# jianing-sun/Mask-YOLO

Hardware: AMD Instinct MI355X
Metric: images/sec fwd+bwd, 224x224 Shapes batch 32, at 1 MI355X (higher is better)
Workload: dtype f32

## Files before the change

### include/myolo_hip_internal.h

```cpp
#ifndef MYOLO_HIP_INTERNAL_H
#define MYOLO_HIP_INTERNAL_H

#include "myolo_hip.h"

#ifdef __cplusplus
extern "C" {
#endif

int myolo_bn_frozen_coeffs_batched(const float* params, const float* stats, const int64_t* table, int nlayers, float* coeffs,
                                   void* stream);

int myolo_bn_act_bwd_frozen_post(const float* dy, const float* a_post, const float* gamma, const float* beta, const float* scale,
                                 float* dx, float* dgamma, float* dbeta, int64_t M, int C, int act,
                                 void* ws, size_t ws_bytes, void* stream);

int myolo_wprep_create(void* arena, size_t arena_bytes, void** handle);
int myolo_wprep_destroy(void* h);
int myolo_wprep_activate(void* h);
int myolo_wprep_count(void* h);
int myolo_wprep_invalidate(void* h);
int myolo_wprep_refresh(void* h, int first, int last, int max_idle, void* stream);
int myolo_wprep_stats(void* h, long long* hits, long long* misses, long long* bytes_used);
int myolo_wprep_overflows(void* h, long long* n);

// ... 81 lines not shown

int myolo_gemm_tn_bf16x6_planes(const float* A, const float* B, float* C, int nruns, const int64_t* rows, const int32_t* nq, int Ka, int N,
                                void* ws, size_t ws_bytes, void* stream);
int myolo_deconv2x2s2_bwd_weight_bf16x6(const float* x, const float* dy, float* dw, int N, int H, int W, int Cin, int Cout, void* ws, size_t ws_bytes,
                                        void* stream);

size_t myolo_wino63_bwd_data_ws_bytes(int N, int Cin, int Cout);
int myolo_wino63_bwd_data_lazybn(const float* y_pre, const float* dy_compact, const int32_t* inv, const float* scale, const float* shift,
                                 const float* ka, const float* kb, int act, const float* w, float* dx, int N, int Cin, int Cout, void* ws,
                                 size_t ws_bytes, void* stream);
int myolo_conv3x3s2_c3_affine_act_fwd(const float* x, const float* w, const float* scale, const float* shift, int act, float* y,
                                      int N, int H, int W, int Cout, void* stream);
size_t myolo_conv3x3s2_c3_bnstats_ws_bytes(int N, int H, int W, int Cout);
int myolo_conv3x3s2_c3_bnstats_fwd(const float* x, const float* w, float* y, const float* gamma, const float* beta, float* mean, float* var,
                                   float* scale, float* shift, float* moving_mean, float* moving_var, int N, int H, int W, int Cout, int phases,
                                   void* ws, size_t ws_bytes, void* stream);
size_t myolo_dwconv3x3_bnstats_ws_bytes(int N, int H, int W, int C, int stride);
int myolo_dwconv3x3_bnstats_fwd(const float* x, const float* in_scale, const float* in_shift, int in_act, const float* w, float* y,
                                const float* gamma, const float* beta, float* mean, float* var, float* scale, float* shift,
                                float* moving_mean, float* moving_var, int N, int H, int W, int C, int stride, int phases,
                                void* ws, size_t ws_bytes, void* stream);
int myolo_dwconv3x3_bwd_weight_affine_in(const float* x, const float* in_scale, const float* in_shift, int in_act, const float* dy, float* dw,
                                         int N, int H, int W, int C, int stride, void* ws, size_t ws_bytes, void* stream);
int    myolo_pwconv1x1_bnstats_ok(int Cin, int Cout);
size_t myolo_pwconv1x1_bnstats_ws_bytes(int64_t M, int Cin, int Cout);
int myolo_pwconv1x1_bnstats_fwd(const float* x, const float* in_scale, const float* in_shift, int in_act, const float* w, float* y,
                                const float* gamma, const float* beta, float* mean, float* var, float* scale, float* shift,
                                float* moving_mean, float* moving_var, int64_t M, int Cin, int Cout, int phases, void* ws, size_t ws_bytes, void* stream);
int myolo_pwconv1x1_bwd_weight_affine_in(const float* x, const float* in_scale, const float* in_shift, int in_act, const float* dy, float* dw,
                                         int64_t M, int Cin, int Cout, void* ws, size_t ws_bytes, void* stream);

int myolo_mask_bce_sel(const float* target_masks, const int32_t* target_class_ids, const float* pred, float loss_weight,
                       float* loss_out, float* dz_sel, int NR, int h, int w, int C, void* ws, size_t ws_bytes, void* stream);
size_t myolo_mask_head_out_bwd_sel_ws_bytes(int NR, int Cin);
int myolo_mask_head_out_bwd_sel(const float* x, const float* w, const float* dz_sel, const int32_t* ids, float* dx, float* dw, float* db,
                                int64_t M, int Cin, int C, int hw, void* ws, size_t ws_bytes, void* stream);

int myolo_stream_copy(const void* src, void* dst, size_t nbytes, int variant, int blocks, void* stream);
int myolo_mfma_probe(int kind, int iters, int blocks, float* out, void* stream);

size_t myolo_conv7x7s2_c3_ws_bytes(int N, int H, int W, int Cout);
int myolo_conv7x7s2_c3_fwd(const float* x, const float* w, const float* bias, float* y, int N, int H, int W, int Cout,
                           void* ws, size_t ws_bytes, void* stream);
int myolo_conv7x7s2_c3_bnstats_fwd(const float* x, const float* w, const float* bias, float* y, const float* gamma, const float* beta, float* mean,
                                   float* var, float* scale, float* shift, float* moving_mean, float* moving_var, int N, int H, int W, int Cout,
                                   void* ws, size_t ws_bytes, void* stream);
// ... 116 lines not shown
```

### mask-yolo_amd/csrc/mem_kernels.hip

```cpp
#include "myolo_common.h"
#include <type_traits>
#include <stdlib.h>
#include <stdarg.h>
#include <string.h>

static thread_local char g_err[512] = "";
extern "C" void myolo_set_error(const char* fmt, ...)
{
    va_list ap;
    va_start(ap, fmt);
    vsnprintf(g_err, sizeof(g_err), fmt, ap);
    va_end(ap);
}
extern "C" const char* myolo_last_error_string(void) { return g_err; }
extern "C" int myolo_version(void) { return 213; }

static MyoloOptions default_options() { MyoloOptions o = {}; o.bn_fused_tf_variance = 1; o.tn_wgs = 224; return o; }
MyoloOptions g_myolo_opt = default_options();
static int* option_slot(const char* name)
{
    static const struct { const char* n; int MyoloOptions::*m; } tab[] = {
        {"gemm_generic", &MyoloOptions::gemm_generic}, {"no_splitk", &MyoloOptions::no_splitk}, {"bf16_no256", &MyoloOptions::bf16_no256},
        {"bf16_force256", &MyoloOptions::bf16_force256}, {"bf16_no_c3", &MyoloOptions::bf16_no_c3}, {"bf16_no_loopn", &MyoloOptions::bf16_no_loopn},
        {"bf16_mask_valu", &MyoloOptions::bf16_mask_valu}, {"bf16_mask_nofin", &MyoloOptions::bf16_mask_nofin},
// ... 316 lines not shown

struct OpStats {
    static constexpr int NV = 2;
    const float* x;
    int C;
    __device__ void operator()(long long r, int c, float4* acc) const
    {
        const float4 v = ld4g(x + r * C + c);
        acc[0].x += v.x; acc[0].y += v.y; acc[0].z += v.z; acc[0].w += v.w;
        acc[1] = f4fma(v, v, acc[1]);
    }
};

struct FinBnStats {
    static constexpr int PAIR = 1;
    const float* gamma;
    const float* beta;
    float *mean, *var, *scale, *shift, *mmean, *mvar;
    double M;
    int fused_tf;
    __device__ void operator()(int, double) const {}
    __device__ void pair(int c, double sum, double sumsq) const
    {
        const double mu = sum / M;
        double vr = sumsq / M - mu * mu;
        if (vr < 0) vr = 0;
        const float rstd = (float)(1.0 / sqrt(vr + (double)BN_EPS_F));
        const float sc = gamma[c] * rstd;
        mean[c] = (float)mu;
        var[c] = (float)vr;
        scale[c] = sc;
        shift[c] = beta[c] - (float)mu * sc;
        if (mmean) {
            float vb = (float)vr;
            if (fused_tf && M > 1.0) vb = vb * ((float)M / ((float)M - 1.0f));
            const float vu = vb * ((float)M / ((float)M - (1.0f + BN_EPS_F)));
            mmean[c] = mmean[c] * BN_MOMENTUM_F + (float)mu * (1.0f - BN_MOMENTUM_F);
            mvar[c] = mvar[c] * BN_MOMENTUM_F + vu * (1.0f - BN_MOMENTUM_F);
        }
    }
};

__global__ void bn_frozen_kernel(const float* gamma, const float* beta, const float* mm, const float* mv,
                                 float* scale, float* shift, int C)
{
    const int c = blockIdx.x * blockDim.x + threadIdx.x;
    if (c >= C) return;
    const float rstd = (float)(1.0 / sqrt((double)mv[c] + (double)BN_EPS_F));
    const float sc = gamma[c] * rstd;
    scale[c] = sc;
    shift[c] = beta[c] - mm[c] * sc;
}

__global__ __launch_bounds__(256) void bn_frozen_batched_kernel(const float* __restrict__ params, const float* __restrict__ stats,
                                                                const long long* __restrict__ table, float* __restrict__ coeffs)
// ... 1111 lines not shown
            double d0 = 0, d1 = 0, d2 = 0, d3 = 0;
            for (int j = 0; j < PX; ++j) {
                const float4 tt = red[j * CQB + tid];
                d0 += tt.x; d1 += tt.y; d2 += tt.z; d3 += tt.w;
            }
            double* o = part + (blk * 9 + v) * C + (cb * CQB + tid) * 4;
            o[0] = d0; o[1] = d1; o[2] = d2; o[3] = d3;
        }
    }
}

template <int S, int CQB>
static void dw_rows_launch(const DwRowsGeom& g, const float* x, const float* w, float* y, int H, int W, int C, DwAffine af, DwFuse fu, hipStream_t s,
                           bool flip = false)
{
    const unsigned xcd = (g.tiles % 8 == 0 && g.tiles >= 64) ? (unsigned)(g.tiles / 8) : 0u;
    const int flags = flip ? 8 : 0;
#define DW_ROWS_GO(MODE, R6) hipLaunchKernelGGL((dw_rows_kernel<S, CQB, MODE, R6>), dim3((unsigned)g.tiles), dim3(256), 0, s, x, w, y, H, W, C, H / S, W / S, g.strips, g.chunks, g.rc, g.ncb, xcd, flags, af, fu)
    if (fu.bw.x) { if constexpr (S == 1) DW_ROWS_GO(3, false); }
    else if (fu.in.scale || fu.stat) { if (fu.in.scale && fu.in.act == MYOLO_ACT_RELU6) DW_ROWS_GO(1, true); else DW_ROWS_GO(1, false); }
    else if (af.scale) { if (af.act == MYOLO_ACT_RELU6) DW_ROWS_GO(2, true); else DW_ROWS_GO(2, false); }
    else DW_ROWS_GO(0, false);
#undef DW_ROWS_GO
}

template <int S>
__global__ __launch_bounds__(256) void dw_bwd_data_kernel(const float* __restrict__ dy, const float* __restrict__ w,
                                                          float* __restrict__ dx, int N, int H, int W, int C, int Ho, int Wo)
{
    const int pt = (S == 1) ? 1 : 0;
    const int cq = C / 4;
    const unsigned e = blockIdx.x * blockDim.x + threadIdx.x;
    if (e >= (unsigned)(W * cq)) return;
    const int ix = e / (unsigned)cq;
    const int c = (e - ix * cq) * 4;
    const int iy = blockIdx.y, n = blockIdx.z;
    float4 acc = f4zero();
#pragma unroll
    for (int ky = 0; ky < 3; ++ky) {
        const int ty = iy + pt - ky;
        if (ty < 0 || (ty % S) != 0) continue;
        const int oy = ty / S;
        if (oy >= Ho) continue;
#pragma unroll
        for (int kx = 0; kx < 3; ++kx) {
            const int tx = ix + pt - kx;
// ... 1547 lines not shown
        double* part = (double*)ws;
        double* tot = (double*)((char*)ws + align256((size_t)nblk * 2 * C * sizeof(double)));
        if (phases & 1) {
            const int rc = dw_fwd_launch(x, w, y, N, H, W, C, stride, DwAffine{nullptr, nullptr, MYOLO_ACT_NONE}, stream, DwFuse{in, part});
            if (rc != MYOLO_OK) return rc;
        }
        if (phases & 2) hipLaunchKernelGGL((colreduce_finish<FinBnStats>), dim3((C + 3) / 4), dim3(256), 0, s, part, tot, nblk, 2 * C, C, fin);
    } else {
        if (phases & 1) {
            const int rc = dw_fwd_launch(x, w, y, N, H, W, C, stride, DwAffine{nullptr, nullptr, MYOLO_ACT_NONE}, stream, DwFuse{in, nullptr});
            if (rc != MYOLO_OK) return rc;
        }
        if (phases & 2) {
            double* part = (double*)ws;
            double* tot = (double*)((char*)ws + align256(col_ws_bytes(M, C, 2)));
            OpStats op{y, C};
            run_colreduce(op, M, C, part, tot, s, fin);
        }
    }
    MYOLO_CHECK_LAUNCH();
    return MYOLO_OK;
}

int myolo_dwconv3x3_bwd_data_bnsums_rows(int N, int H, int W, int C, int stride)
{
    if (N <= 0 || (C & 3)) return 0;
    if (stride == 1) return dw_rows_ok(H, W, C) ? dw_rows_geom(N, H, W, C, 1).nblk : 0;
    if (stride != 2 || (H & 1) || (W & 1)) return 0;
    const int cq = C / 4;
    const long long total = (long long)N * (H / 2) * (W / 2) * cq;
    if (cq > 256 || (256 % cq) != 0 || total >= (1ll << 31) * 256) return 0;
    if (cq > 64) return 0;
    return (int)((total + 255) / 256);
}

static int dw_bwd_data_impl(const float* dy, const float* w, float* dx, int N, int H, int W, int C, int stride, DwBnBwd bw, void* stream);

int myolo_dwconv3x3_bwd_data(const float* dy, const float* w, float* dx, int N, int H, int W, int C, int stride, void* stream)
{
    return dw_bwd_data_impl(dy, w, dx, N, H, W, C, stride, DwBnBwd{nullptr, nullptr, nullptr, nullptr, nullptr, 0, nullptr}, stream);
}

int myolo_dwconv3x3_bwd_data_bnsums(const float* dy, const float* w, float* dx, int N, int H, int W, int C, int stride, const float* xbn,
                                    const float* scale, const float* shift, const float* mean, const float* var, int act, double* part, int rows,
                                    void* stream)
{
// ... 357 lines not shown
```

### mask-yolo_amd/myolo/_ext.py

```python
import ctypes
import os

import torch

_LIB = None
_HERE = os.path.dirname(os.path.abspath(__file__))
LIB_PATH = os.environ.get("MYOLO_LIB") or os.path.join(_HERE, "_lib", "libmyolo_hip.so")

P, I, L, F, Z, D = ctypes.c_void_p, ctypes.c_int, ctypes.c_int64, ctypes.c_float, ctypes.c_size_t, ctypes.c_double

SIGS = {
    "myolo_conv3x3s2_c3_fwd": [P, P, P, I, I, I, I, P],
    "myolo_conv3x3s2_c3_affine_act_fwd": [P, P, P, P, I, P, I, I, I, I, P],
    "myolo_conv3x3s2_c3_bwd_weight": [P, P, P, I, I, I, I, P, Z, P],
    "myolo_dwconv3x3_fwd": [P, P, P, I, I, I, I, I, P],
    "myolo_dwconv3x3_affine_act_fwd": [P, P, P, P, I, P, I, I, I, I, I, P],
    "myolo_dwconv3x3_bwd_data": [P, P, P, I, I, I, I, I, P],
    "myolo_dwconv3x3_bwd_data_bnsums": [P, P, P, I, I, I, I, I, P, P, P, P, P, I, P, I, P],
    "myolo_bn_act_bwd_from_partials": [P, P, P, P, P, P, P, P, P, L, I, I, P, I, P, Z, P],
    "myolo_dwconv3x3_bwd_weight": [P, P, P, I, I, I, I, I, P, Z, P],
    "myolo_pwconv1x1_fwd": [P, P, P, P, L, I, I, P, Z, P],
    "myolo_pwconv1x1_affine_act_fwd": [P, P, P, P, I, P, L, I, I, P, Z, P],
    "myolo_bn_frozen_coeffs_batched": [P, P, P, I, P, P],
    "myolo_pwconv1x1_bwd_data": [P, P, P, L, I, I, P, Z, P],
# ... 62 lines not shown
    "myolo_conv3x3_wino_bwd_data_lazybn": [P, P, P, P, P, P, P, I, P, P, I, I, I, I, I, P, Z, P],
    "myolo_conv3x3_wino_bwd_weight_lazybn": [P, P, P, P, P, P, P, P, I, P, I, I, I, I, I, P, Z, P],
    "myolo_wino_input_transform_roialign": [P, P, P, P, I, I, I, I, I, I, I, P],
    "myolo_pack_weights_bf16": [P, I, I, I, P, P, P, P, P, P, P, P],
    "myolo_crop_and_resize_bf16_fwd": [P, P, P, P, I, I, I, I, I, I, I, P],
    "myolo_conv3x3_bf16_fwd": [P, P, P, P, I, I, I, I, I, I, P],
    "myolo_deconv2x2s2_bf16_fwd": [P, P, P, P, I, I, I, I, I, I, P],
    "myolo_deconv2x2s2_mask_bf16_fwd": [P, P, P, P, P, P, I, I, I, I, I, I, P, Z, P],
    "myolo_mask_head_out_bf16_fwd": [P, P, P, P, L, I, I, P],
    "myolo_mask_head_out_bwd": [P, P, P, P, P, P, L, I, I, P, Z, P],
    "myolo_mask_bce": [P, P, P, F, P, P, I, I, I, I, P, Z, P],
    "myolo_mask_bce_sel": [P, P, P, F, P, P, I, I, I, I, P, Z, P],
    "myolo_mask_head_out_bwd_sel": [P, P, P, P, P, P, P, L, I, I, I, P, Z, P],
    "myolo_adam_step": [P, P, P, P, L, F, F, F, F, F, P],
    "myolo_grad_sumsq": [P, P, L, F, F, P, P, P],
    "myolo_adamw_ema_step": [P, P, P, P, P, P, L, P, F, F, F, F, F, F, F, F, P],
    "myolo_swap_f32": [P, P, L, P],
    "myolo_matmul_f32": [P, P, P, L, I, I, I, I, P, Z, P],
    "myolo_stream_copy": [P, P, Z, I, I, P],
    "myolo_mfma_probe": [I, I, I, P, P],
    "myolo_conv3x3s2_c3_bnstats_fwd": [P, P, P, P, P, P, P, P, P, P, P, I, I, I, I, I, P, Z, P],
    "myolo_dwconv3x3_bnstats_fwd": [P, P, P, I, P, P, P, P, P, P, P, P, P, P, I, I, I, I, I, I, P, Z, P],
    "myolo_dwconv3x3_bwd_weight_affine_in": [P, P, P, I, P, P, I, I, I, I, I, P, Z, P],
    "myolo_pwconv1x1_bnstats_fwd": [P, P, P, I, P, P, P, P, P, P, P, P, P, P, L, I, I, I, P, Z, P],
    "myolo_pwconv1x1_bwd_weight_affine_in": [P, P, P, I, P, P, L, I, I, P, Z, P],
    "myolo_gemm_tn_bf16x6_planes": [P, P, P, I, P, P, I, I, P, Z, P],
    "myolo_deconv2x2s2_bwd_weight_bf16x6": [P, P, P, I, I, I, I, I, P, Z, P],
    "myolo_gather_groups_affine_act": [P, P, P, P, I, P, P, I, L, I, P],
    "myolo_add_inplace": [P, P, L, P],
    "myolo_conv7x7s2_c3_fwd": [P, P, P, P, I, I, I, I, P, Z, P],
    "myolo_conv7x7s2_c3_bnstats_fwd": [P, P, P, P, P, P, P, P, P, P, P, P, I, I, I, I, P, Z, P],
    "myolo_conv7x7s2_c3_affine_act_fwd": [P, P, P, P, P, I, P, I, I, I, I, P, Z, P],
    "myolo_conv7x7s2_c3_bwd_weight": [P, P, P, P, I, I, I, I, P, Z, P],
    "myolo_maxpool3x3s2_fwd": [P, P, P, I, P, P, I, I, I, I, P],
    "myolo_maxpool3x3s2_bwd": [P, P, P, I, I, I, I, P],
    "myolo_gather_s2": [P, P, I, I, I, I, P],
    "myolo_scatter_s2": [P, P, P, I, I, I, I, P],
    "myolo_residual_fwd": [P, P, P, P, P, P, P, L, I, P],
    "myolo_residual_bwd": [P, P, P, L, P],
    "myolo_fill": [P, F, L, P],
    "myolo_u8_to_unit_f32": [P, P, L, P],
    "myolo_augment_batch": [P, P, P, P, D, P, P, P, P, P, P, P, I, I, I, I, I, I, I, P, Z, P],
    "myolo_mosaic_batch": [P, P, P, P, P, P, D, P, P, P, P, P, P, P, P, I, I, I, I, I, I, I, P, Z, P],
    "myolo_copy_paste_batch": [P, P, P, P, P, P, P, P, P, P, P, P, P, I, I, I, I, I, I, I, P, Z, P],
    "myolo_segment_masks": [P, P, P, P, P, P, P, P, P, P, I, I, I, I, P],
    "myolo_resize_images_u8": [P, Z, P, P, P, P, I, I, I, P, Z, P],
# ... 16 lines not shown
    global _LIB
    if _LIB is not None:
        return _LIB
    if not os.path.exists(LIB_PATH):
        raise RuntimeError("libmyolo_hip.so not built (%s): run `python __graft_entry__.py` "
                           "(hipcc --offload-arch=gfx950); there is no fallback path" % LIB_PATH)
    lib = ctypes.CDLL(LIB_PATH)
    for name, argtypes in SIGS.items():
        fn = getattr(lib, name)
        fn.argtypes = argtypes
        fn.restype = ctypes.c_int
    lib.myolo_version.restype = ctypes.c_int
    lib.myolo_last_error_string.restype = ctypes.c_char_p
    lib.myolo_workspace_bytes.argtypes = [L, I, I]
    lib.myolo_workspace_bytes.restype = Z
    lib.myolo_conv3x3_wino_ws_bytes.argtypes = [I, I, I, I, I, I]
    lib.myolo_conv3x3_wino_ws_bytes.restype = Z
    lib.myolo_matmul_f32_ws_bytes.argtypes = [I, I, I, I]
    lib.myolo_matmul_f32_ws_bytes.restype = Z
    lib.myolo_conv3x3s2_c3_bnstats_ws_bytes.argtypes = [I, I, I, I]
    lib.myolo_conv3x3s2_c3_bnstats_ws_bytes.restype = Z
    lib.myolo_dwconv3x3_bnstats_ws_bytes.argtypes = [I, I, I, I, I]
    lib.myolo_dwconv3x3_bnstats_ws_bytes.restype = Z
    lib.myolo_dwconv3x3_bwd_weight_ws_bytes.argtypes = [I, I, I, I, I]
    lib.myolo_dwconv3x3_bwd_weight_ws_bytes.restype = Z
    lib.myolo_pwconv1x1_bnstats_ws_bytes.argtypes = [L, I, I]
    lib.myolo_pwconv1x1_bnstats_ws_bytes.restype = Z
    lib.myolo_pwconv1x1_bnstats_ok.argtypes = [I, I]
    lib.myolo_pwconv1x1_bnstats_ok.restype = I
    lib.myolo_wino_plane_elems.argtypes = [I, I, I, I]
    lib.myolo_wino_plane_elems.restype = Z
    lib.myolo_wino_u_elems.argtypes = [I, I]
    lib.myolo_wino_u_elems.restype = Z
    lib.myolo_wino63_u_elems.argtypes = [I, I]
    lib.myolo_wino63_u_elems.restype = Z
    lib.myolo_wino63_plane_elems.argtypes = [I, I]
    lib.myolo_wino63_plane_elems.restype = Z
    lib.myolo_wino63_bwd_data_ws_bytes.argtypes = [I, I, I]
    lib.myolo_wino63_bwd_data_ws_bytes.restype = Z
    lib.myolo_conv3x3_wino63_ws_bytes.argtypes = [I, I, I, I]
    lib.myolo_conv3x3_wino63_ws_bytes.restype = Z
    lib.myolo_wino63_bwd_weight_ws_bytes.argtypes = [I, I, I]
    lib.myolo_wino63_bwd_weight_ws_bytes.restype = Z
    for fn in (lib.myolo_wino63_bwd_data_from_v_ws_bytes, lib.myolo_wino63_bwd_weight_from_q_ws_bytes):
        fn.argtypes = [I, I, I]
        fn.restype = Z
# ... 20 lines not shown
    lib.myolo_conv7x7s2_c3_ws_bytes.restype = Z
    lib.myolo_augment_batch_ws_bytes.argtypes = [I, I]
    lib.myolo_augment_batch_ws_bytes.restype = Z
    lib.myolo_mosaic_batch_ws_bytes.argtypes = [I, I]
    lib.myolo_mosaic_batch_ws_bytes.restype = Z
    lib.myolo_copy_paste_batch_ws_bytes.argtypes = [I, I]
    lib.myolo_copy_paste_batch_ws_bytes.restype = Z
    lib.myolo_resize_images_ws_bytes.argtypes = [I]
    lib.myolo_resize_images_ws_bytes.restype = Z
    lib.myolo_rle_masks_ws_bytes.argtypes = [I, I, I]
    lib.myolo_rle_masks_ws_bytes.restype = Z
    lib.myolo_contour_masks_ws_bytes.argtypes = [I, I, I, I, L]
    lib.myolo_contour_masks_ws_bytes.restype = Z
    lib.myolo_anchor_kmeans_ws_bytes.argtypes = [L, I]
    lib.myolo_anchor_kmeans_ws_bytes.restype = Z
    lib.myolo_wprep_refresh.argtypes = [P, I, I, I, P]
    lib.myolo_wprep_refresh.restype = I
    _LIB = lib
    return lib


def exported_symbols():
    return list(SIGS) + ["myolo_version", "myolo_last_error_string", "myolo_workspace_bytes", "myolo_conv3x3_wino_ws_bytes", "myolo_wino_plane_elems", "myolo_wino_u_elems", "myolo_wino63_u_elems", "myolo_wino63_plane_elems", "myolo_wino63_ok", "myolo_wino63_bwd_data_ws_bytes", "myolo_wino63_bwd_weight_ws_bytes", "myolo_wino63_bwd_data_from_v_ws_bytes", "myolo_wino63_bwd_weight_from_q_ws_bytes", "myolo_wino63_output_transform_bn_ws_bytes", "myolo_conv3x3_wino63_ws_bytes", "myolo_matmul_f32_ws_bytes", "myolo_conv3x3s2_c3_bnstats_ws_bytes", "myolo_dwconv3x3_bnstats_ws_bytes", "myolo_dwconv3x3_bwd_weight_ws_bytes",
                              "myolo_pwconv1x1_bnstats_ws_bytes", "myolo_pwconv1x1_bnstats_ok",
                              "myolo_deconv2x2s2_mask_ws_bytes", "myolo_wino_output_transform_bn_ws_bytes", "myolo_mask_head_out_bwd_sel_ws_bytes",
                              "myolo_dwconv3x3_bwd_data_bnsums_rows", "myolo_wprep_create", "myolo_wprep_destroy", "myolo_wprep_activate", "myolo_wprep_invalidate", "myolo_wprep_count", "myolo_wprep_refresh",
                              "myolo_conv7x7s2_c3_ws_bytes", "myolo_augment_batch_ws_bytes", "myolo_mosaic_batch_ws_bytes", "myolo_copy_paste_batch_ws_bytes",
                              "myolo_resize_images_ws_bytes",
                              "myolo_rle_masks_ws_bytes", "myolo_contour_masks_ws_bytes", "myolo_anchor_kmeans_ws_bytes"]


def ptr(t):
    if t is None:
        return None
    assert t.is_cuda and t.is_contiguous(), "C-ABI needs contiguous device tensors"
    return t.data_ptr()


def stream():
    return torch.cuda.current_stream().cuda_stream


def call(name, *args):
    lib = load()
    rc = getattr(lib, name)(*args)
    if rc != 0:
        raise RuntimeError("%s failed (%d): %s" % (name, rc, lib.myolo_last_error_string().decode()))
# ... 191 lines not shown
def anchor_kmeans_ws_bytes(n, runs):
    return int(load().myolo_anchor_kmeans_ws_bytes(int(n), int(runs)))


def workspace_bytes(rows, cin, cout):
    return int(load().myolo_workspace_bytes(int(rows), int(cin), int(cout)))


def wino_ws_bytes(n, h, w, cin, cout, which):
    return int(load().myolo_conv3x3_wino_ws_bytes(int(n), int(h), int(w), int(cin), int(cout), int(which)))


PRODUCTS_NATIVE, PRODUCTS_BF16X6 = 0, 1


def conv1_bnstats_ws_bytes(n, h, w, cout):
    return int(load().myolo_conv3x3s2_c3_bnstats_ws_bytes(int(n), int(h), int(w), int(cout)))


def dw_bnstats_ws_bytes(n, h, w, c, stride):
    return int(load().myolo_dwconv3x3_bnstats_ws_bytes(int(n), int(h), int(w), int(c), int(stride)))


def dw_bwd_weight_ws_bytes(n, h, w, c, stride):
    return int(load().myolo_dwconv3x3_bwd_weight_ws_bytes(int(n), int(h), int(w), int(c), int(stride)))


def pw_bnstats_ws_bytes(m, cin, cout):
    return int(load().myolo_pwconv1x1_bnstats_ws_bytes(int(m), int(cin), int(cout)))


def pw_bnstats_ok(cin, cout):
    return bool(load().myolo_pwconv1x1_bnstats_ok(int(cin), int(cout)))


def matmul_ws_bytes(k, n, b_is_nk, products):
    return int(load().myolo_matmul_f32_ws_bytes(int(k), int(n), int(b_is_nk), int(products)))


def wino_u_elems(cin, cout):
    return int(load().myolo_wino_u_elems(int(cin), int(cout)))


def dw_bwd_data_bnsums_rows(n, h, w, c, stride):
    return int(load().myolo_dwconv3x3_bwd_data_bnsums_rows(int(n), int(h), int(w), int(c), int(stride)))

# ... 52 lines not shown
```

### mask-yolo_amd/myolo/engine.py

```python
import contextlib
import gc
import os
import threading
import time

import numpy as np
import torch

from . import _ext as X

ACT_NONE, ACT_RELU, ACT_RELU6 = 0, 1, 2

BACKBONE_BLOCKS = [(64, 1), (64, 2), (128, 1), (256, 2), (256, 1), (512, 1)]
YOLO_BLOCKS = [(512, 2), (512, 1), (512, 1), (512, 1), (512, 1), (512, 1), (1024, 2), (1024, 1)]
MASK_FILTERS = 256
RESNET_STAGES = [(2, "abc", (64, 64, 256), 1), (3, "abcd", (128, 128, 512), 2), (4, "abcdef", (256, 256, 1024), 2), (5, "abc", (512, 512, 2048), 2)]
RESNET_C4_STAGE = 3
RESNET_MAX_MASK_ROIS = 32 * 7 * 7 * 3


def resnet_check_size(n_images, h, w, n_box):
    rois = int(n_images) * (int(h) // 32) * (int(w) // 32) * int(n_box)
    if rois > RESNET_MAX_MASK_ROIS:
        raise ValueError("BACKBONE='resnet50': %d images of %dx%d with N_BOX=%d give %d mask-head ROIs per launch; only up to %d are supported "
# ... 436 lines not shown
        self._rle_pin = None
        self._contour_verts = None
        self._contour_ws = None
        self._contour_pin = None
        self._render_args = None
        self._render_pin = None
        self._select_pin = None
        self._cap_stream = None
        self._fm_stream = None
        self.infer_fork_feature_map = False
        self._fork_now = None
        self._ws_main = Workspace(self.dev, on_realloc=lambda: self._drop_graphs(0))
        self._side = None
        self._yolo_stream = _shared_stream(self.dev, "yolo_head_bwd")
        self._yolo_side = _Side(self._yolo_stream, Workspace(self.dev))
        self.yolo_bwd_early = -1
        self.exchange_active = False
        self._wgrad_stream = _shared_stream(self.dev, "weight_gradients")
        self._wgrad_side = _Side(self._wgrad_stream, Workspace(self.dev))
        self._twg_stream = self._wgrad_stream
        self.lazy_bn1_bwd = True
        self.fold_frozen_bn = True
        self.fuse_trunk_bn = bool(getattr(cfg, "FUSE_TRUNK_BN", True))
        self._fz_table = None
        self.anchors = torch.tensor(np.asarray(cfg.ANCHORS, np.float32), device=self.dev)
        self.class_weights = torch.tensor(np.asarray(cfg.CLASS_WEIGHTS, np.float32), device=self.dev)
        self.adam_t = 0
        self.flat_ema = None
        self._opt_stats = None
        self._opt_partials = None
        self._opt_stats_pin = None
        self.tape = {}
        self.proposals_hook = None
        self.tape_hook = None
        self.on_bucket_ready = None
        self.before_optimizer = None
        self.grad_scale = 1.0
        self.conv3x3_algo = getattr(cfg, "CONV3X3_ALGO", "auto")
        if self.conv3x3_algo not in ("auto", "direct", "winograd"):
            raise ValueError("CONV3X3_ALGO must be 'auto', 'direct' or 'winograd' (got %r)" % (self.conv3x3_algo,))
        self.wino_tiles = getattr(cfg, "WINOGRAD_TILES", "f43")
        if self.wino_tiles not in ("f43", "f63"):
            raise ValueError("WINOGRAD_TILES must be 'f43' or 'f63' (got %r)" % (self.wino_tiles,))
        self.fp32_matmul = getattr(cfg, "FP32_MATMUL", "native")
        if self.fp32_matmul not in ("native", "bf16x6"):
            raise ValueError("FP32_MATMUL must be 'native' or 'bf16x6' (got %r)" % (self.fp32_matmul,))
# ... 111 lines not shown
        if side is not None and side.pending:
            torch.cuda.current_stream().wait_stream(side.stream)
            side.pending = False

    def _release(self, bucket, side):
        if not self.on_bucket_ready:
            return
        if side.pending:
            with self._on(side):
                self.on_bucket_ready(bucket)
        else:
            self.on_bucket_ready(bucket)

    def _call_timed(self, tag, name, *args):
        if tag not in self.timed_tags:
            return X.call(name, *args)
        st = torch.cuda.current_stream()
        e0, e1 = torch.cuda.Event(enable_timing=True), torch.cuda.Event(enable_timing=True)
        e0.record(st)
        X.call(name, *args)
        e1.record(st)
        self.timings.setdefault(tag, []).append((e0, e1))

    def _call_conv_then_finish(self, tag, name, args):
        if tag not in self.timed_tags:
            return X.call(name, *args, 3, *self._wsargs(), X.stream())
        self._call_timed(tag, name, *args, 1, *self._wsargs(), X.stream())
        X.call(name, *args, 2, *self._wsargs(), X.stream())

    def kernel_ms(self, tag):
        torch.cuda.synchronize()
        ev = self.timings.get(tag, [])
        return sum(a.elapsed_time(b) for a, b in ev) / max(1, len(ev)), len(ev)

    def bn_act_fwd(self, name, y, act, batch_stats):
        M, C = y.shape
        scale, shift = self.bnbuf[name][2:4]
        self.tape[name] = (y, act, batch_stats)
        a = self._new(M, C)
        if batch_stats:
            X.call("myolo_bn_stats", X.ptr(y), *self._bn_args(name), M, C, *self._wsargs(), X.stream())
        elif C % 4 == 0 and 256 % (C // 4) == 0:
            X.call("myolo_bn_frozen_apply_act", X.ptr(y), X.ptr(self.p[name + "/gamma"]), X.ptr(self.p[name + "/beta"]),
                   X.ptr(self.s[name + "/moving_mean"]), X.ptr(self.s[name + "/moving_variance"]), X.ptr(scale), X.ptr(shift), X.ptr(a),
                   M, C, act, X.stream())
            return a
        else:
# ... 132 lines not shown
    def _in_args(self, a):
        if self._is_lazy(a):
            _, y, bn = a
            buf = self.bnbuf[bn]
            return X.ptr(y), X.ptr(buf[2]), X.ptr(buf[3]), ACT_RELU6
        return X.ptr(a), None, None, ACT_NONE

    def _materialize(self, a):
        if not self._is_lazy(a):
            return a
        _, y, bn = a
        buf = self.bnbuf[bn]
        out = self._new(*y.shape)
        X.call("myolo_bn_apply_act", X.ptr(y), X.ptr(buf[2]), X.ptr(buf[3]), X.ptr(out), y.shape[0], y.shape[1], ACT_RELU6, X.stream())
        return out

    def _bn_args(self, name):
        buf = self.bnbuf[name]
        return (X.ptr(self.p[name + "/gamma"]), X.ptr(self.p[name + "/beta"]), X.ptr(buf[0]), X.ptr(buf[1]), X.ptr(buf[2]), X.ptr(buf[3]),
                X.ptr(self.s[name + "/moving_mean"]), X.ptr(self.s[name + "/moving_variance"]))

    def _block_fusable(self, C, Co):
        return self.fuse_trunk_bn and C % 4 == 0 and X.pw_bnstats_ok(C, Co)

    def dw_block_fwd(self, bid, a, shape, stride, train):
        N, H, W, C = shape
        Ho, Wo = H // stride, W // stride
        dwn, pwn = "conv_dw_%d" % bid, "conv_pw_%d" % bid
        if not train and self.fold_frozen_bn:
            sc, sh = self._frozen_affine(dwn + "_bn")
            ad = self._new(N * Ho * Wo, C)
            self._call_timed("dw%d_fwd" % bid, "myolo_dwconv3x3_affine_act_fwd", X.ptr(a), X.ptr(self.p[dwn + "/depthwise_kernel"]), sc, sh,
                             ACT_RELU6, X.ptr(ad), N, H, W, C, stride, X.stream())
            Co = self.p[pwn + "/kernel"].shape[3]
            sc, sh = self._frozen_affine(pwn + "_bn")
            ap = self._new(N * Ho * Wo, Co)
            self._call_timed("pw%d_fwd" % bid, "myolo_pwconv1x1_affine_act_fwd", X.ptr(ad), X.ptr(self.p[pwn + "/kernel"]), sc, sh,
                             ACT_RELU6, X.ptr(ap), N * Ho * Wo, C, Co, *self._wsargs(), X.stream())
            return ap, (N, Ho, Wo, Co)
        Co = self.p[pwn + "/kernel"].shape[3]
        M = N * Ho * Wo
        if train and self._block_fusable(C, Co):
            y = self._new(M, C)
            self.ws.ensure(max(X.dw_bnstats_ws_bytes(N, H, W, C, stride), X.pw_bnstats_ws_bytes(M, C, Co)))
            self._call_conv_then_finish("dw%d_fwd" % bid, "myolo_dwconv3x3_bnstats_fwd", (*self._in_args(a), X.ptr(self.p[dwn + "/depthwise_kernel"]), X.ptr(y),
                                        *self._bn_args(dwn + "_bn"), N, H, W, C, stride))
            self.tape[dwn + "_bn"] = (y, ACT_RELU6, True)
            ad = ("lazy", y, dwn + "_bn")
            y2 = self._new(M, Co)
            self._call_conv_then_finish("pw%d_fwd" % bid, "myolo_pwconv1x1_bnstats_fwd", (*self._in_args(ad), X.ptr(self.p[pwn + "/kernel"]), X.ptr(y2),
                                        *self._bn_args(pwn + "_bn"), M, C, Co))
            self.tape[pwn + "_bn"] = (y2, ACT_RELU6, True)
            self.tape["blk%d" % bid] = (a, shape, stride, ad)
            return ("lazy", y2, pwn + "_bn"), (N, Ho, Wo, Co)
        a = self._materialize(a)
        y = self._new(M, C)
        self._call_timed("dw%d_fwd" % bid, "myolo_dwconv3x3_fwd", X.ptr(a), X.ptr(self.p[dwn + "/depthwise_kernel"]), X.ptr(y),
                         N, H, W, C, stride, X.stream())
        ad = self.bn_act_fwd(dwn + "_bn", y, ACT_RELU6, train)
        y2 = self._new(M, Co)
        self._call_timed("pw%d_fwd" % bid, "myolo_pwconv1x1_fwd", X.ptr(ad), X.ptr(self.p[pwn + "/kernel"]), None, X.ptr(y2), M, C, Co,
                         *self._wsargs(), X.stream())
        ap = self.bn_act_fwd(pwn + "_bn", y2, ACT_RELU6, train)
        self.tape["blk%d" % bid] = (a, shape, stride, ad)
        return ap, (N, Ho, Wo, Co)

    def join_trunk_wgrad(self):
        self._join(self._wgrad_side)
        self._join(self._yolo_side)

    def dw_block_bwd(self, bid, da, next_bn=None, wside=None):
        a, shape, stride, ad = self.tape["blk%d" % bid]
        N, H, W, C = shape
        Ho, Wo = H // stride, W // stride
# ... 1724 lines not shown
```

Measured before the change: 1676.

## Fuse previous pointwise BN finish into depthwise conv with per-channel LDS-resident owner kernel

Adds a depthwise-conv forward kernel where each workgroup owns a channel pair or quad across the whole batch. It loads the full slab into 128KB LDS, reduces the previous pointwise layer's BN statistics, applies BN+ReLU6 in place, runs the 3x3 depthwise conv, and computes this layer's BN stats in the same launch. The engine leaves the previous pw BN unfinished (phase 1 only) for small late-stage blocks, which removes the separate finish kernels and extra passes over activations. The cost is low parallelism, since there is one workgroup per channel group, and it depends on large dynamic LDS being available.

```diff
diff --git a/include/myolo_hip_internal.h b/include/myolo_hip_internal.h
--- a/include/myolo_hip_internal.h
+++ b/include/myolo_hip_internal.h
@@ -127,6 +127,11 @@
                                 void* ws, size_t ws_bytes, void* stream);
 int myolo_dwconv3x3_bwd_weight_affine_in(const float* x, const float* in_scale, const float* in_shift, int in_act, const float* dy, float* dw,
                                          int N, int H, int W, int C, int stride, void* ws, size_t ws_bytes, void* stream);
+int myolo_dw_owner_ok(int N, int H, int W, int C, int stride);
+int myolo_dw_owner_fwd(const float* x, const float* x_gamma, const float* x_beta, float* x_mean, float* x_var, float* x_scale, float* x_shift,
+                       float* x_moving_mean, float* x_moving_var, const float* w, float* y, const float* gamma, const float* beta, float* mean,
+                       float* var, float* scale, float* shift, float* moving_mean, float* moving_var, int N, int H, int W, int C, int stride,
+                       void* stream);
 int    myolo_pwconv1x1_bnstats_ok(int Cin, int Cout);
 size_t myolo_pwconv1x1_bnstats_ws_bytes(int64_t M, int Cin, int Cout);
 int myolo_pwconv1x1_bnstats_fwd(const float* x, const float* in_scale, const float* in_shift, int in_act, const float* w, float* y,
diff --git a/mask-yolo_amd/csrc/mem_kernels.hip b/mask-yolo_amd/csrc/mem_kernels.hip
--- a/mask-yolo_amd/csrc/mem_kernels.hip
+++ b/mask-yolo_amd/csrc/mem_kernels.hip
@@ -362,15 +362,21 @@
     __device__ void operator()(int, double) const {}
     __device__ void pair(int c, double sum, double sumsq) const
     {
+        float sc, sh;
+        pair(c, sum, sumsq, sc, sh);
+    }
+    __device__ void pair(int c, double sum, double sumsq, float& sc, float& sh) const
+    {
         const double mu = sum / M;
         double vr = sumsq / M - mu * mu;
         if (vr < 0) vr = 0;
         const float rstd = (float)(1.0 / sqrt(vr + (double)BN_EPS_F));
-        const float sc = gamma[c] * rstd;
+        sc = gamma[c] * rstd;
+        sh = beta[c] - (float)mu * sc;
         mean[c] = (float)mu;
         var[c] = (float)vr;
         scale[c] = sc;
-        shift[c] = beta[c] - (float)mu * sc;
+        shift[c] = sh;
         if (mmean) {
             float vb = (float)vr;
             if (fused_tf && M > 1.0) vb = vb * ((float)M / ((float)M - 1.0f));
@@ -1528,6 +1534,147 @@
     else if (af.scale) { if (af.act == MYOLO_ACT_RELU6) DW_ROWS_GO(2, true); else DW_ROWS_GO(2, false); }
     else DW_ROWS_GO(0, false);
 #undef DW_ROWS_GO
+}
+
+#define DW_OWNER_THREADS 1024
+#define DW_OWNER_LDS_BYTES (128 * 1024)
+#define DW_OWNER_NP (DW_OWNER_LDS_BYTES / 16 / DW_OWNER_THREADS)
+#define DW_OWNER_TW(S, L) ((L) == 2 ? 7 : ((S) == 1 ? 4 : 2))
+
+template <int L> struct dw_owner_vec;
+template <> struct dw_owner_vec<4> { typedef float type __attribute__((ext_vector_type(4))); };
+template <> struct dw_owner_vec<2> { typedef float type __attribute__((ext_vector_type(2))); };
+
+template <int L, class T>
+__device__ __forceinline__ void dw_owner_reduce(T s, T q, double* wred, double* out)
+{
+    double d[2 * L];
+#pragma unroll
+    for (int k = 0; k < L; ++k) { d[k] = (double)s[k]; d[L + k] = (double)q[k]; }
+#pragma unroll
+    for (int off = 32; off >= 1; off >>= 1) {
+#pragma unroll
+        for (int k = 0; k < 2 * L; ++k) d[k] += __shfl_xor(d[k], off, 64);
+    }
+    const int tid = threadIdx.x;
+    if ((tid & 63) == 0) {
+#pragma unroll
+        for (int k = 0; k < 2 * L; ++k) wred[(tid >> 6) * 2 * L + k] = d[k];
+    }
+    __syncthreads();
+    if (tid < 2 * L) {
+        double t = 0;
+        for (int wv = 0; wv < DW_OWNER_THREADS / 64; ++wv) t += wred[wv * 2 * L + tid];
+        out[tid] = t;
+    }
+    __syncthreads();
+}
+
+template <int S, int L>
+__global__ __launch_bounds__(DW_OWNER_THREADS) void dw_owner_fwd_kernel(const float* __restrict__ x, const float* __restrict__ w,
+                                                                        float* __restrict__ y, int N, int H, int W, int C, FinBnStats fx,
+                                                                        FinBnStats fy)
+{
+    typedef typename dw_owner_vec<L>::type T;
+    extern __shared__ float4 dw_owner_lds[];
+    T* slab = reinterpret_cast<T*>(dw_owner_lds);
+    __shared__ double wred[DW_OWNER_THREADS / 64 * 2 * L];
+    __shared__ double tot[2 * L];
+    __shared__ float coef[2 * L];
+    const int tid = threadIdx.x;
+    const unsigned nwg = (unsigned)(C / L);
+    unsigned b = blockIdx.x;
+    if ((nwg & 7u) == 0) b = (b & 7u) * (nwg >> 3) + (b >> 3);
+    const int c = (int)b * L;
+    const int P = N * H * W;
+    constexpr int PAD = (S == 1) ? 1 : 0;
+    const int Ho = H / S, Wo = W / S;
+    const T zero = T(0.f);
+    T wv[9];
+#pragma unroll
+    for (int k = 0; k < 9; ++k) wv[k] = *reinterpret_cast<const T*>(w + k * C + c);
+    T s = zero, q = zero;
+    {
+        const float* xp = x + c;
+        T v[DW_OWNER_NP];
+#pragma unroll
+        for (int k = 0; k < DW_OWNER_NP; ++k) {
+            const int i = tid + k * DW_OWNER_THREADS;
+            v[k] = *reinterpret_cast<const T*>(xp + (long long)min(i, P - 1) * C);
+        }
+#pragma unroll
+        for (int k = 0; k < DW_OWNER_NP; ++k) {
+            const int i = tid + k * DW_OWNER_THREADS;
+            if (i < P) slab[i] = v[k];
+            const T u = i < P ? v[k] : zero;
+            s += u;
+            q = __builtin_elementwise_fma(u, u, q);
+        }
+    }
+    dw_owner_reduce<L>(s, q, wred, tot);
+    if (tid < L) {
+        float sc, sh;
+        fx.pair(c + tid, tot[tid], tot[L + tid], sc, sh);
+        coef[tid] = sc;
+        coef[L + tid] = sh;
+    }
+    __syncthreads();
+    {
+        T sc, sh;
+#pragma unroll
+        for (int k = 0; k < L; ++k) { sc[k] = coef[k]; sh[k] = coef[L + k]; }
+        for (int i = tid; i < P; i += DW_OWNER_THREADS) {
+            T a = __builtin_elementwise_fma(slab[i], sc, sh);
+#pragma unroll
+            for (int k = 0; k < L; ++k) a[k] = __builtin_amdgcn_fmed3f(a[k], 0.f, 6.f);
+            slab[i] = a;
+        }
+    }
+    __syncthreads();
+    s = zero; q = zero;
+    {
+        constexpr int TW = DW_OWNER_TW(S, L), NC = (TW - 1) * S + 3;
+        float* yp = y + c;
+        const unsigned strips = (unsigned)((Wo + TW - 1) / TW);
+        const unsigned per_img = (unsigned)Ho * strips;
+        const int items = N * (int)per_img;
+        for (int it = tid; it < items; it += DW_OWNER_THREADS) {
+            const unsigned n = (unsigned)it / per_img, r = (unsigned)it % per_img;
+            const int oy = (int)(r / strips), ox0 = (int)(r % strips) * TW;
+            const T* img = slab + (int)n * H * W;
+            T acc[TW];
+#pragma unroll
+            for (int j = 0; j < TW; ++j) acc[j] = zero;
+#pragma unroll
+            for (int ky = 0; ky < 3; ++ky) {
+                const int iy = oy * S + ky - PAD;
+                const bool yin = iy >= 0 && iy < H;
+                const T* row = img + (yin ? iy : 0) * W;
+#pragma unroll
+                for (int k = 0; k < NC; ++k) {
+                    const int ix = ox0 * S + k - PAD;
+                    const bool in = yin && ix >= 0 && ix < W;
+                    const T v = in ? row[ix] : zero;
+#pragma unroll
+                    for (int kx = 0; kx < 3; ++kx) {
+                        if ((k - kx) >= 0 && ((k - kx) % S) == 0 && (k - kx) / S < TW)
+                            acc[(k - kx) / S] = __builtin_elementwise_fma(v, wv[ky * 3 + kx], acc[(k - kx) / S]);
+                    }
+                }
+            }
+            float* yrow = yp + ((long long)((int)n * Ho + oy) * Wo + ox0) * C;
+#pragma unroll
+            for (int j = 0; j < TW; ++j) {
+                if (ox0 + j < Wo) {
+                    *reinterpret_cast<T*>(yrow + (long long)j * C) = acc[j];
+                    s += acc[j];
+                    q = __builtin_elementwise_fma(acc[j], acc[j], q);
+                }
+            }
+        }
+    }
+    dw_owner_reduce<L>(s, q, wred, tot);
+    if (tid < L) fy.pair(c + tid, tot[tid], tot[L + tid]);
 }
 
 template <int S>
@@ -3121,6 +3268,61 @@
     return MYOLO_OK;
 }
 
+int myolo_dw_owner_ok(int N, int H, int W, int C, int stride)
+{
+    if (N <= 0 || H <= 0 || W <= 0 || C <= 0 || (C & 3) || (stride != 1 && stride != 2)) return 0;
+    if (stride == 2 && ((H & 1) || (W & 1))) return 0;
+    return (long long)N * H * W * 16 <= DW_OWNER_LDS_BYTES ? 1 : 0;
+}
+
+int myolo_dw_owner_fwd(const float* x, const float* x_gamma, const float* x_beta, float* x_mean, float* x_var, float* x_scale, float* x_shift,
+                       float* x_moving_mean, float* x_moving_var, const float* w, float* y, const float* gamma, const float* beta, float* mean,
+                       float* var, float* scale, float* shift, float* moving_mean, float* moving_var, int N, int H, int W, int C, int stride,
+                       void* stream)
+{
+    MYOLO_REQUIRE(x && x_gamma && x_beta && x_mean && x_var && x_scale && x_shift && w && y && gamma && beta && mean && var && scale && shift,
+                  "dw_owner_fwd: bad arguments");
+    MYOLO_REQUIRE(N > 0 && H > 0 && W > 0 && C > 0 && (C & 3) == 0 && (stride == 1 || stride == 2), "dw_owner_fwd: bad arguments");
+    MYOLO_REQUIRE(stride == 1 || ((H & 1) == 0 && (W & 1) == 0), "dw_owner_fwd: stride 2 needs even H, W");
+    MYOLO_REQUIRE(myolo_dw_owner_ok(N, H, W, C, stride), "dw_owner_fwd: a channel quad's slab of %lld bytes (N*H*W*16) is over the %d-byte LDS budget",
+                  (long long)N * H * W * 16, DW_OWNER_LDS_BYTES);
+    MYOLO_REQUIRE((((uintptr_t)x | (uintptr_t)w | (uintptr_t)y) & 15) == 0, "dw_owner_fwd: needs 16-byte aligned x, w, y");
+    hipStream_t s = (hipStream_t)stream;
+    const int fused_tf = g_myolo_opt.bn_fused_tf_variance;
+    const FinBnStats fx{x_gamma, x_beta, x_mean, x_var, x_scale, x_shift, x_moving_mean, x_moving_var, (double)N * H * W, fused_tf};
+    const FinBnStats fy{gamma, beta, mean, var, scale, shift, moving_mean, moving_var, (double)N * (H / stride) * (W / stride), fused_tf};
+    static int cus_dev[64] = {};
+    int dev = 0;
+    (void)hipGetDevice(&dev);
+    int& cus = cus_dev[dev & 63];
+    if (!cus) {
+        const void* kernels[4] = {(const void*)dw_owner_fwd_kernel<1, 4>, (const void*)dw_owner_fwd_kernel<2, 4>, (const void*)dw_owner_fwd_kernel<1, 2>,
+                                  (const void*)dw_owner_fwd_kernel<2, 2>};
+        for (const void* k : kernels) {
+            if (hipFuncSetAttribute(k, hipFuncAttributeMaxDynamicSharedMemorySize, DW_OWNER_LDS_BYTES) != hipSuccess) {
+                (void)hipGetLastError();
+                myolo_set_error("dw_owner_fwd: this device does not allow %d bytes of dynamic LDS", DW_OWNER_LDS_BYTES);
+                return MYOLO_EINVAL;
+            }
+        }
+        int n = 0;
+        if (hipDeviceGetAttribute(&n, hipDeviceAttributeMultiprocessorCount, dev) != hipSuccess || n <= 0) n = 256;
+        cus = n;
+    }
+    const bool quads = C / 4 >= cus;
+    const size_t lds = (size_t)N * H * W * (quads ? 16 : 8);
+    const dim3 grid(quads ? C / 4 : C / 2), block(DW_OWNER_THREADS);
+    if (stride == 1) {
+        if (quads) hipLaunchKernelGGL((dw_owner_fwd_kernel<1, 4>), grid, block, lds, s, x, w, y, N, H, W, C, fx, fy);
+        else hipLaunchKernelGGL((dw_owner_fwd_kernel<1, 2>), grid, block, lds, s, x, w, y, N, H, W, C, fx, fy);
+    } else {
+        if (quads) hipLaunchKernelGGL((dw_owner_fwd_kernel<2, 4>), grid, block, lds, s, x, w, y, N, H, W, C, fx, fy);
+        else hipLaunchKernelGGL((dw_owner_fwd_kernel<2, 2>), grid, block, lds, s, x, w, y, N, H, W, C, fx, fy);
+    }
+    MYOLO_CHECK_LAUNCH();
+    return MYOLO_OK;
+}
+
 int myolo_dwconv3x3_bwd_data_bnsums_rows(int N, int H, int W, int C, int stride)
 {
     if (N <= 0 || (C & 3)) return 0;
diff --git a/mask-yolo_amd/myolo/_ext.py b/mask-yolo_amd/myolo/_ext.py
--- a/mask-yolo_amd/myolo/_ext.py
+++ b/mask-yolo_amd/myolo/_ext.py
@@ -108,6 +108,7 @@
     "myolo_conv3x3s2_c3_bnstats_fwd": [P, P, P, P, P, P, P, P, P, P, P, I, I, I, I, I, P, Z, P],
     "myolo_dwconv3x3_bnstats_fwd": [P, P, P, I, P, P, P, P, P, P, P, P, P, P, I, I, I, I, I, I, P, Z, P],
     "myolo_dwconv3x3_bwd_weight_affine_in": [P, P, P, I, P, P, I, I, I, I, I, P, Z, P],
+    "myolo_dw_owner_fwd": [P, P, P, P, P, P, P, P, P, P, P, P, P, P, P, P, P, P, P, I, I, I, I, I, P],
     "myolo_pwconv1x1_bnstats_fwd": [P, P, P, I, P, P, P, P, P, P, P, P, P, P, L, I, I, I, P, Z, P],
     "myolo_pwconv1x1_bwd_weight_affine_in": [P, P, P, I, P, P, L, I, I, P, Z, P],
     "myolo_gemm_tn_bf16x6_planes": [P, P, P, I, P, P, I, I, P, Z, P],
@@ -170,6 +171,8 @@
     lib.myolo_conv3x3s2_c3_bnstats_ws_bytes.restype = Z
     lib.myolo_dwconv3x3_bnstats_ws_bytes.argtypes = [I, I, I, I, I]
     lib.myolo_dwconv3x3_bnstats_ws_bytes.restype = Z
+    lib.myolo_dw_owner_ok.argtypes = [I, I, I, I, I]
+    lib.myolo_dw_owner_ok.restype = I
     lib.myolo_dwconv3x3_bwd_weight_ws_bytes.argtypes = [I, I, I, I, I]
     lib.myolo_dwconv3x3_bwd_weight_ws_bytes.restype = Z
     lib.myolo_pwconv1x1_bnstats_ws_bytes.argtypes = [L, I, I]
@@ -236,7 +239,7 @@
 
 def exported_symbols():
     return list(SIGS) + ["myolo_version", "myolo_last_error_string", "myolo_workspace_bytes", "myolo_conv3x3_wino_ws_bytes", "myolo_wino_plane_elems", "myolo_wino_u_elems", "myolo_wino63_u_elems", "myolo_wino63_plane_elems", "myolo_wino63_ok", "myolo_wino63_bwd_data_ws_bytes", "myolo_wino63_bwd_weight_ws_bytes", "myolo_wino63_bwd_data_from_v_ws_bytes", "myolo_wino63_bwd_weight_from_q_ws_bytes", "myolo_wino63_output_transform_bn_ws_bytes", "myolo_conv3x3_wino63_ws_bytes", "myolo_matmul_f32_ws_bytes", "myolo_conv3x3s2_c3_bnstats_ws_bytes", "myolo_dwconv3x3_bnstats_ws_bytes", "myolo_dwconv3x3_bwd_weight_ws_bytes",
-                              "myolo_pwconv1x1_bnstats_ws_bytes", "myolo_pwconv1x1_bnstats_ok",
+                              "myolo_pwconv1x1_bnstats_ws_bytes", "myolo_pwconv1x1_bnstats_ok", "myolo_dw_owner_ok",
                               "myolo_deconv2x2s2_mask_ws_bytes", "myolo_wino_output_transform_bn_ws_bytes", "myolo_mask_head_out_bwd_sel_ws_bytes",
                               "myolo_dwconv3x3_bwd_data_bnsums_rows", "myolo_wprep_create", "myolo_wprep_destroy", "myolo_wprep_activate", "myolo_wprep_invalidate", "myolo_wprep_count", "myolo_wprep_refresh",
                               "myolo_conv7x7s2_c3_ws_bytes", "myolo_augment_batch_ws_bytes", "myolo_mosaic_batch_ws_bytes", "myolo_copy_paste_batch_ws_bytes",
@@ -474,6 +477,10 @@
     return int(load().myolo_dwconv3x3_bnstats_ws_bytes(int(n), int(h), int(w), int(c), int(stride)))
 
 
+def dw_owner_ok(n, h, w, c, stride):
+    return bool(load().myolo_dw_owner_ok(int(n), int(h), int(w), int(c), int(stride)))
+
+
 def dw_bwd_weight_ws_bytes(n, h, w, c, stride):
     return int(load().myolo_dwconv3x3_bwd_weight_ws_bytes(int(n), int(h), int(w), int(c), int(stride)))
 
diff --git a/mask-yolo_amd/myolo/engine.py b/mask-yolo_amd/myolo/engine.py
--- a/mask-yolo_amd/myolo/engine.py
+++ b/mask-yolo_amd/myolo/engine.py
@@ -482,6 +482,9 @@
         self.lazy_bn1_bwd = True
         self.fold_frozen_bn = True
         self.fuse_trunk_bn = bool(getattr(cfg, "FUSE_TRUNK_BN", True))
+        self.dw_owner = bool(getattr(cfg, "DW_OWNER", True))
+        self.dw_owner_max_pixels = int(getattr(cfg, "DW_OWNER_MAX_PIXELS", 8192))
+        self._bn_open = None
         self._fz_table = None
         self.anchors = torch.tensor(np.asarray(cfg.ANCHORS, np.float32), device=self.dev)
         self.class_weights = torch.tensor(np.asarray(cfg.CLASS_WEIGHTS, np.float32), device=self.dev)
@@ -639,7 +642,9 @@
         e1.record(st)
         self.timings.setdefault(tag, []).append((e0, e1))
 
-    def _call_conv_then_finish(self, tag, name, args):
+    def _call_conv_then_finish(self, tag, name, args, finish=True):
+        if not finish:
+            return self._call_timed(tag, name, *args, 1, *self._wsargs(), X.stream())
         if tag not in self.timed_tags:
             return X.call(name, *args, 3, *self._wsargs(), X.stream())
         self._call_timed(tag, name, *args, 1, *self._wsargs(), X.stream())
@@ -818,6 +823,17 @@
 
     def _block_fusable(self, C, Co):
         return self.fuse_trunk_bn and C % 4 == 0 and X.pw_bnstats_ok(C, Co)
+
+    def _dw_owner_block(self, bid, shape):
+        blocks = BACKBONE_BLOCKS + YOLO_BLOCKS
+        if not self.dw_owner or bid < 2 or bid > len(blocks) or bid == len(BACKBONE_BLOCKS) + 1:
+            return False
+        N, H, W, C = shape
+        Co = self.p["conv_pw_%d/kernel" % bid].shape[3]
+        stride = blocks[bid - 1][1]
+        pixels = N * H * W + N * (H // stride) * (W // stride)
+        prev_fused = self._block_fusable(self.p["conv_pw_%d/kernel" % (bid - 1)].shape[2], C)
+        return pixels <= self.dw_owner_max_pixels and prev_fused and self._block_fusable(C, Co) and X.dw_owner_ok(N, H, W, C, stride)
 
     def dw_block_fwd(self, bid, a, shape, stride, train):
         N, H, W, C = shape
@@ -839,13 +855,23 @@
         if train and self._block_fusable(C, Co):
             y = self._new(M, C)
             self.ws.ensure(max(X.dw_bnstats_ws_bytes(N, H, W, C, stride), X.pw_bnstats_ws_bytes(M, C, Co)))
-            self._call_conv_then_finish("dw%d_fwd" % bid, "myolo_dwconv3x3_bnstats_fwd", (*self._in_args(a), X.ptr(self.p[dwn + "/depthwise_kernel"]), X.ptr(y),
-                                        *self._bn_args(dwn + "_bn"), N, H, W, C, stride))
+            if self._dw_owner_block(bid, shape):
+                if not (self._is_lazy(a) and a[2] == self._bn_open):
+                    raise RuntimeError("dw_block_fwd: block %d expects the open BatchNorm of conv_pw_%d (got %r)" % (bid, bid - 1, self._bn_open))
+                self._bn_open = None
+                self._call_timed("dw%d_fwd" % bid, "myolo_dw_owner_fwd", X.ptr(a[1]), *self._bn_args(a[2]), X.ptr(self.p[dwn + "/depthwise_kernel"]),
+                                 X.ptr(y), *self._bn_args(dwn + "_bn"), N, H, W, C, stride, X.stream())
+            else:
+                self._call_conv_then_finish("dw%d_fwd" % bid, "myolo_dwconv3x3_bnstats_fwd", (*self._in_args(a), X.ptr(self.p[dwn + "/depthwise_kernel"]), X.ptr(y),
+                                            *self._bn_args(dwn + "_bn"), N, H, W, C, stride))
             self.tape[dwn + "_bn"] = (y, ACT_RELU6, True)
             ad = ("lazy", y, dwn + "_bn")
             y2 = self._new(M, Co)
+            leave_open = self._dw_owner_block(bid + 1, (N, Ho, Wo, Co))
             self._call_conv_then_finish("pw%d_fwd" % bid, "myolo_pwconv1x1_bnstats_fwd", (*self._in_args(ad), X.ptr(self.p[pwn + "/kernel"]), X.ptr(y2),
-                                        *self._bn_args(pwn + "_bn"), M, C, Co))
+                                        *self._bn_args(pwn + "_bn"), M, C, Co), finish=not leave_open)
+            if leave_open:
+                self._bn_open = pwn + "_bn"
             self.tape[pwn + "_bn"] = (y2, ACT_RELU6, True)
             self.tape["blk%d" % bid] = (a, shape, stride, ad)
             return ("lazy", y2, pwn + "_bn"), (N, Ho, Wo, Co)
```

Result: no change. 1679 (median of 6 runs) (+0.2%).
